# Peterande/SAST

Hardware: AMD Instinct MI355X
Metric: frames/sec (B=4) SAST backbone fwd+bwd, 1Mpx 640x360 (higher is better)
Workload: dtype f32; 1 GPU; 1Mpx 640x360 (padded 384x640) full SAST backbone + PAFPN, fwd+bwd + AdamW, B=4/GPU, binary events (rand>0.5), random-init, AMP=0.0002; global_batch=4, seq_len=1, parallelism=dp1, hipgraph=True, library=sast_amd/libsast_hip.so, product_library=True, segmented_backward_overlap=False, deferred_weight_gradients=False, backward_cuts=3, dw_discard_TIMING_PROBE_gradients_invalid=False, collective_ranks=1, collective_ranks_verified=1, gradient_bytes_per_rank=67663616, sync_batchnorm=False, event_dtype=int32, grads_finite=True

## Files before the change

### sast_amd/csrc/gemm.cuh

```cuda
#pragma once
#include <type_traits>
#include <hip/hip_ext.h>
#include "common.cuh"
#include "../../include/sast_hip.h"

#if defined(SAST_TL_ENABLE) && !defined(SAST_TL)
static __device__ unsigned long long sast_tl_buf[8 * 8192];
#define SAST_TL(k)                                                                                          \
  do {                                                                                                      \
    const unsigned bid_ = blockIdx.x;                                                                       \
    if (threadIdx.x == 0 && bid_ < 8192) sast_tl_buf[bid_ * 8 + (k)] = wall_clock64();                      \
    if (threadIdx.x == 0 && bid_ < 8192 && (k) == 0) sast_tl_buf[bid_ * 8 + 7] = __smid();                 \
  } while (0)
#define SAST_TL_JOB(j) do { if (threadIdx.x == 0 && blockIdx.x < 8192) sast_tl_buf[blockIdx.x * 8 + 6] = (j); } while (0)
#endif
#ifndef SAST_TL
#define SAST_TL(k)
#endif
#ifndef SAST_TL_JOB
#define SAST_TL_JOB(j)
#endif
#ifndef SAST_TLF
#define SAST_TLF_DECL
#define SAST_TLF(k)
// ... 739 lines not shown
  const int remap = xcd_remap_enabled() && nb >= 16;
  const int grid = remap ? (nb + 7) / 8 * 8 : nb;
  if (prof_enabled()) {
    hipEvent_t e0, e1;
    prof_kernel_events(__PRETTY_FUNCTION__, T::G, M, NJ, R, dM, dR, st, &e0, &e1, LoaderSrcBytes<LA>::get(la), LoaderSrcBytes<LB>::get(lb));
    SAST_EXT_LAUNCH((gemm_kernel<T, LA, LB, EP, false>), dim3(grid + ep_side_blocks(ep)), dim3(T::NT), 0, st, e0, e1, 0, la, lb, ep, M, NJ,
                          R, dM, dR, (float*)nullptr, 1, remap);
  } else {
    SAST_LAUNCH((gemm_kernel<T, LA, LB, EP, false>), dim3(grid + ep_side_blocks(ep)), dim3(T::NT), 0, st, la, lb, ep, M, NJ, R, dM, dR,
                       (float*)nullptr, 1, remap);
  }
  SAST_CHECK_LAUNCH();
  return SAST_OK;
}

template <class T, class LA, class LB, class EP>
inline int launch_gemm_split(const LA& la, const LB& lb, const EP& ep, int M, int NJ, int R, const int* dR,
                             int splits, float* colsum, hipStream_t st) {
  if (M <= 0 || NJ <= 0 || R <= 0) return SAST_OK;
  if (colsum != nullptr && LA::RC && GemmSmem<T, LA, LB>::PSA) return SAST_EINVAL;
  if (!gemm_span_ok<T>(la, lb, M, NJ, R)) return SAST_EINVAL;
  const int nb = ((M + T::BM - 1) / T::BM) * ((NJ + T::BJ - 1) / T::BJ);
  if (splits < 1) splits = 1;
  const int remap = xcd_remap_enabled() && nb * splits >= 16;
  const int grid = remap ? (nb * splits + 7) / 8 * 8 : nb * splits;
  if (prof_enabled()) {
    hipEvent_t e0, e1;
    prof_kernel_events(__PRETTY_FUNCTION__, T::G, M, NJ, R, nullptr, dR, st, &e0, &e1, LoaderSrcBytes<LA>::get(la), LoaderSrcBytes<LB>::get(lb));
    SAST_EXT_LAUNCH((gemm_kernel<T, LA, LB, EP, true>), dim3(grid), dim3(T::NT), 0, st, e0, e1, 0, la, lb, ep, M, NJ, R,
                          (const int*)nullptr, dR, colsum, splits, remap);
  } else {
    SAST_LAUNCH((gemm_kernel<T, LA, LB, EP, true>), dim3(grid), dim3(T::NT), 0, st, la, lb, ep, M, NJ, R,
                       (const int*)nullptr, dR, colsum, splits, remap);
  }
  SAST_CHECK_LAUNCH();
  return SAST_OK;
}

inline int gemm_grid(int ntile, int nsplit, int& remap) {
  const int n = ntile * nsplit;
  remap = xcd_remap_enabled() && n >= 16;
  return remap ? (n + 7) / 8 * 8 : n;
}
void prof_kernel_events2(const char* tag, double flops_static, int G1, int M1, int NJ1, int R1, const int* dM1, const int* dR1, int G2,
                         int M2, int NJ2, int R2, const int* dM2, const int* dR2, hipStream_t st, hipEvent_t* e0, hipEvent_t* e1,
                         double a1_cap = -1.0, double b1_cap = -1.0, double a2_cap = -1.0, double b2_cap = -1.0);

template <class TS, class LA1, class LB1, class EP1, class TP, class LA2, class LB2, class EP2>
inline int launch_gemm_dual(const LA1& la1, const LB1& lb1, const EP1& ep1, int M1, int NJ1, int R1, const int* dR1, int splits,
                            float* colsum, const LA2& la2, const LB2& lb2, const EP2& ep2, int M2, int NJ2, int R2, const int* dM2,
                            hipStream_t st) {
  using J1 = GemmJob<TS, LA1, LB1, EP1, true>;
  using J2 = GemmJob<TP, LA2, LB2, EP2, false>;
  if (colsum != nullptr && LA1::RC && GemmSmem<TS, LA1, LB1>::PSA) return SAST_EINVAL;
  if (!gemm_span_ok<TS>(la1, lb1, M1, NJ1, R1) || !gemm_span_ok<TP>(la2, lb2, M2, NJ2, R2)) return SAST_EINVAL;
  if (splits < 1) splits = 1;
  const int nt1 = ((M1 + TS::BM - 1) / TS::BM) * ((NJ1 + TS::BJ - 1) / TS::BJ);
  const int nt2 = ((M2 + TP::BM - 1) / TP::BM) * ((NJ2 + TP::BJ - 1) / TP::BJ);
  int r1, r2;
  int n1 = gemm_grid(nt1, splits, r1);
  const int n2 = gemm_grid(nt2, 1, r2);
  if (r2 && (n1 & 7)) n1 = (n1 + 7) / 8 * 8;
  const J1 a{la1, lb1, ep1, M1, NJ1, R1, nullptr, dR1, colsum, splits, r1};
  const J2 b{la2, lb2, ep2, M2, NJ2, R2, dM2, nullptr, nullptr, 1, r2};
  constexpr int NTHREADS = TS::NT > TP::NT ? TS::NT : TP::NT;
  if (prof_enabled()) {
    hipEvent_t e0, e1;
    prof_kernel_events2(__PRETTY_FUNCTION__, 0.0, TS::G, M1, NJ1, R1, nullptr, dR1, TP::G, M2, NJ2, R2, dM2, nullptr, st, &e0, &e1,
                        LoaderSrcBytes<LA1>::get(la1), LoaderSrcBytes<LB1>::get(lb1), LoaderSrcBytes<LA2>::get(la2), LoaderSrcBytes<LB2>::get(lb2));
    SAST_EXT_LAUNCH((gemm_dual_kernel<J1, J2>), dim3(n1 + n2 + ep_side_blocks(ep2)), dim3(NTHREADS), 0, st, e0, e1, 0, a, b, n1);
  } else {
    SAST_LAUNCH((gemm_dual_kernel<J1, J2>), dim3(n1 + n2 + ep_side_blocks(ep2)), dim3(NTHREADS), 0, st, a, b, n1);
  }
  SAST_CHECK_LAUNCH();
  return SAST_OK;
}

using TileBig   = Tile<128, 128, 2, 2, 1>;
using TileMid   = Tile<64, 128, 2, 2, 1>;
using TileSmall = Tile<64, 64, 2, 2, 1>;
using TileSmallK2 = Tile<64, 64, 2, 2, 1, 16, 2>;
using TileSmallK4 = Tile<64, 64, 2, 2, 1, 16, 4>;
using TileSplitR = Tile<64, 64, 2, 1, 1, 16, 2>;
using TileThinK4  = Tile<32, 64, 1, 2, 1, 16, 4>;
using TileTinyK8 = Tile<32, 32, 1, 1, 1, 16, 8>;
using TileTiny  = Tile<32, 32, 1, 1, 1>;
using TileN64   = Tile<128, 64, 4, 1, 1>;
using TileG2    = Tile<64, 128, 2, 2, 2>;
using TileG2Big = Tile<128, 128, 2, 2, 2>;
using TileG2Tiny = Tile<32, 64, 1, 1, 2>;
using TileG2K2  = Tile<64, 64, 2, 1, 2, 16, 2>;
using TileG2K4  = Tile<32, 64, 1, 1, 2, 16, 4>;
using TileG4K4  = Tile<32, 128, 1, 1, 4, 16, 4>;
using TileG4    = Tile<64, 128, 2, 1, 4, 16, 1, 2, 2>;
using TileG4Big = Tile<128, 128, 4, 1, 4>;
using TileG4Tiny = Tile<32, 128, 1, 1, 4>;
using TileG3    = Tile<64, 96, 2, 1, 3>;
using TileG3K4  = Tile<32, 96, 1, 1, 3, 16, 4>;

__host__ __device__ inline int small_div_mul(int d) { return 65536 / d + 1; }


static __device__ __attribute__((aligned(16))) float sast_zero_page[4];
__device__ __forceinline__ float4 ldz(bool ok, const float* valid) { return ld4(ok ? valid : sast_zero_page); }
__device__ __forceinline__ float ldz1(bool ok, const void* valid) {
  return *reinterpret_cast<const float*>(ok ? valid : (const void*)sast_zero_page);
}
#define SAST_DEFAULT_FINISH \
  __device__ __forceinline__ float4 finish(float4 v, float, bool) const { return v; }

struct LdRows {
  static constexpr bool RC = true, BUFFERED = true;
  const float* p; int ld; const int* idx; int nsrc = 0;
  unsigned long long span_bytes(int I, int, int R) const { return 4ull * ((unsigned long long)((idx ? nsrc : I) - 1) * ld + R); }
  struct Ctx { unsigned row; };
  using Desc = BufDesc;
  __device__ __forceinline__ Desc desc(int) const { return Desc{make_buf(p, BUF_MAX_BYTES)}; }
  __device__ __forceinline__ Ctx prep(int i, int Ieff) const {
    const bool ok = i < Ieff;
    const int ii = ok ? i : 0;
    return Ctx{ok ? 4u * (unsigned)(idx ? idx[ii] : ii) * (unsigned)ld : BUF_INVALID};
  }
  __device__ __forceinline__ void load(const Desc& d, const Ctx& c, int r0, int off, int Rl, int, float4& v, float& aux, bool& ok) const {
    ok = off < Rl - r0;
    v = ldb(d.d, ok ? (c.row + 4u * off) + 4u * r0 : BUF_INVALID);
    aux = 0.f;
  }
  SAST_DEFAULT_FINISH
};
struct LdRows2 {
  static constexpr bool RC = true;
  const float* p1; int ld1; int R1; const float* p2; int ld2;
  struct Ctx { const float* a; const float* b; bool ok; };
  __device__ __forceinline__ Ctx prep(int i, int Ieff) const {
    const bool ok = i < Ieff;
    const int ii = ok ? i : 0;
    return Ctx{p1 + (size_t)ii * ld1, p2 ? p2 + (size_t)ii * ld2 - R1 : p1 + (size_t)ii * ld1, ok};
  }
  __device__ __forceinline__ void load(const Ctx& c, int r, int Reff, float4& v, float& aux, bool& ok) const {
    const bool second = r >= R1;
    ok = c.ok && r < Reff && (!second || p2 != nullptr);
    const float* q = second ? c.b : c.a;
    v = ldz(ok, q + r);
    aux = 0.f;
  }
  SAST_DEFAULT_FINISH
};
struct LdRowsT {
  static constexpr bool RC = false, BUFFERED = true;
  const float* p; int ld;
  unsigned long long span_bytes(int, int, int R) const { return 4ull * (unsigned long long)(R + BUF_SPAN_SLACK_ROWS) * ld; }
  struct Ctx { unsigned col; };
  using Desc = BufDesc;
  __device__ __forceinline__ Desc desc(int Rl) const { return Desc{make_buf(p, 4u * (unsigned)Rl * (unsigned)ld)}; }
  __device__ __forceinline__ Ctx prep(int i, int Ieff) const { return Ctx{i < Ieff ? 4u * i : BUF_INVALID}; }
  __device__ __forceinline__ Ctx prep(int j, int, int NJ) const { return Ctx{j < NJ ? 4u * j : BUF_INVALID}; }
  __device__ __forceinline__ void load(const Desc& d, const Ctx& c, int r0, int off, int, int, float4& v, float& aux, bool& ok) const {
    ok = true;
    v = ldb(d.d, (c.col + 4u * (unsigned)(off * ld)) + 4u * (unsigned)(r0 * ld));
    aux = 0.f;
  }
  SAST_DEFAULT_FINISH
};
struct LdRowsTG {
  static constexpr bool RC = false, BUFFERED = true;
  const float* p; int ld; const int* idx; int nsrc;
// ... 590 lines not shown
```

### sast_amd/csrc/gemm_dispatch.cuh

```cuda
#pragma once
#include <cstdlib>
#include "gemm.cuh"

namespace sast {

using TileAutoThin = TileThinK4;
using TileAutoK2 = TileSmallK2;
using TileAutoK1 = TileSmall;

inline bool gemm_pair_enabled() { return SAST_KNOB("SAST_GEMM_PAIR", 1) != 0; }
inline int pair_tn_blocks() { return SAST_KNOB("SAST_TN_BLOCKS", 768); }
inline int pair_ks_min_r() { return SAST_KNOB("SAST_KS_MINR", 256); }
inline int pair_thin_nb() { return SAST_KNOB("SAST_THIN_NB", 384); }
inline int pair_ks_nb() { return SAST_KNOB("SAST_KS_NB", 1000000); }
inline int tiny_nb() { return SAST_KNOB("SAST_TINY_NB", 128); }
inline bool use_tiny(int M, int NJ, int R) { return (long)((M + 31) / 32) * ((NJ + 63) / 64) <= tiny_nb() && R >= 512; }

template <class LA, class LB, class EP>
int gemm_auto(const LA& la, const LB& lb, const EP& ep, int M, int NJ, int R, const int* dM, hipStream_t st, int R_tile = 0) {
  const long nb = (long)((M + 63) / 64) * ((NJ + 63) / 64);
  const int Rt = R_tile > 0 ? R_tile : R;
  if (!dM && use_tiny(M, NJ, Rt)) return launch_gemm<TileTinyK8>(la, lb, ep, M, NJ, R, dM, nullptr, st);
  if (nb <= pair_thin_nb() && Rt >= pair_ks_min_r()) return launch_gemm<TileAutoThin>(la, lb, ep, M, NJ, R, dM, nullptr, st);
  if (nb <= pair_ks_nb() && Rt >= pair_ks_min_r()) return launch_gemm<TileAutoK2>(la, lb, ep, M, NJ, R, dM, nullptr, st);
  return launch_gemm<TileAutoK1>(la, lb, ep, M, NJ, R, dM, nullptr, st);
}
template <class LA, class LB, class EP>
int gemm_auto(const LA& la, const LB& lb, const EP& ep, int M, int NJ, int R, hipStream_t st) {
  return gemm_auto(la, lb, ep, M, NJ, R, nullptr, st);
}

inline int pair_tn_blocks_conv() { return SAST_KNOB("SAST_TN_BLOCKS_PAIRED_CONV", 192); }
inline int pair_tn_blocks_1x1() { return SAST_KNOB("SAST_TN_BLOCKS_PAIRED_1X1", 192); }
inline int pair_tn_blocks_paired() { return SAST_KNOB("SAST_TN_BLOCKS_PAIRED", 192); }
inline int pair_tn_blocks_small() { return SAST_KNOB("SAST_TN_BLOCKS_PAIRED_SMALL", 0); }
inline int pair_tn_small_tiles() { return SAST_KNOB("SAST_TN_SMALL_TILES", 4); }

inline int tn_splits(int Mo, int NJ, int R, int target = 0) {
  const int nb = ((Mo + 63) / 64) * ((NJ + 63) / 64);
  if (target <= 0) target = pair_tn_blocks();
  int splits = (target + nb - 1) / nb;
  const int max_splits = (R + 127) / 128;
  if (splits > max_splits) splits = max_splits;
  return splits < 1 ? 1 : splits;
}

template <class LA, class LB>
int gemm_tn(const LA& la, const LB& lb, float* out, int ldc, int Mo, int NJ, int R, const int* dR, float* colsum, hipStream_t st) {
  return launch_gemm_split<TileSplitR>(la, lb, EpAtomic{out, ldc}, Mo, NJ, R, dR, tn_splits(Mo, NJ, R), colsum, st);
}
template <class LA, class LB>
int gemm_tn(const LA& la, const LB& lb, float* out, int ldc, int Mo, int NJ, int R, hipStream_t st) {
  return gemm_tn(la, lb, out, ldc, Mo, NJ, R, nullptr, nullptr, st);
}

template <class LA1, class LB1, class EP1, class LA2, class LB2, class EP2>
int gemm_pair_ep(const LA1& la1, const LB1& lb1, const EP1& ep1, int Mo, int NJ1, int R1, const int* dR1, float* colsum,
                 const LA2& la2, const LB2& lb2, const EP2& ep2, int M2, int NJ2, int R2, const int* dM2, hipStream_t st, int tn_target = 0,
                 int R2_tile = 0);
template <class LA1, class LB1, class LA2, class LB2, class EP2>
int gemm_pair(const LA1& la1, const LB1& lb1, float* out, int ldc, int Mo, int NJ1, int R1, const int* dR1, float* colsum,
              const LA2& la2, const LB2& lb2, const EP2& ep2, int M2, int NJ2, int R2, const int* dM2, hipStream_t st, int tn_target = 0,
              int R2_tile = 0) {
  return gemm_pair_ep(la1, lb1, EpAtomic{out, ldc}, Mo, NJ1, R1, dR1, colsum, la2, lb2, ep2, M2, NJ2, R2, dM2, st, tn_target, R2_tile);
}
template <class LA1, class LB1, class EP1, class LA2, class LB2, class EP2>
int gemm_pair_ep(const LA1& la1, const LB1& lb1, const EP1& ep1, int Mo, int NJ1, int R1, const int* dR1, float* colsum,
                 const LA2& la2, const LB2& lb2, const EP2& ep2, int M2, int NJ2, int R2, const int* dM2, hipStream_t st, int tn_target,
                 int R2_tile) {
  const long nb2 = (long)((M2 + 63) / 64) * ((NJ2 + 63) / 64);
  const int R2t = R2_tile > 0 ? R2_tile : R2;
  const bool thin = nb2 <= pair_thin_nb() && R2t >= pair_ks_min_r(), k2 = nb2 <= pair_ks_nb() && R2t >= pair_ks_min_r();
  const int nb1 = ((Mo + 63) / 64) * ((NJ1 + 63) / 64);
  if (gemm_pair_enabled() && pair_tn_blocks_small() > 0 && nb1 <= pair_tn_small_tiles()) tn_target = pair_tn_blocks_small();
  const int splits = tn_splits(Mo, NJ1, R1, gemm_pair_enabled() ? (tn_target > 0 ? tn_target : pair_tn_blocks_paired()) : 0);
  if (!gemm_pair_enabled() || Mo <= 0 || NJ1 <= 0 || R1 <= 0 || M2 <= 0 || NJ2 <= 0 || R2 <= 0) {
    int rc = launch_gemm_split<TileSplitR>(la1, lb1, ep1, Mo, NJ1, R1, dR1, splits, colsum, st);
    if (rc) return rc;
    if (thin) return launch_gemm<TileAutoThin>(la2, lb2, ep2, M2, NJ2, R2, dM2, nullptr, st);
    if (k2) return launch_gemm<TileAutoK2>(la2, lb2, ep2, M2, NJ2, R2, dM2, nullptr, st);
    return launch_gemm<TileAutoK1>(la2, lb2, ep2, M2, NJ2, R2, dM2, nullptr, st);
  }
  if (thin)
    return launch_gemm_dual<TileSplitR, LA1, LB1, EP1, TileAutoThin, LA2, LB2, EP2>(la1, lb1, ep1, Mo, NJ1, R1, dR1, splits, colsum, la2, lb2,
                                                                                      ep2, M2, NJ2, R2, dM2, st);
  if (k2)
    return launch_gemm_dual<TileSplitR, LA1, LB1, EP1, TileAutoK2, LA2, LB2, EP2>(la1, lb1, ep1, Mo, NJ1, R1, dR1, splits, colsum, la2, lb2,
                                                                                       ep2, M2, NJ2, R2, dM2, st);
  return launch_gemm_dual<TileSplitR, LA1, LB1, EP1, TileAutoK1, LA2, LB2, EP2>(la1, lb1, ep1, Mo, NJ1, R1, dR1, splits, colsum, la2, lb2, ep2,
                                                                                   M2, NJ2, R2, dM2, st);
}

}
```

### sast_amd/csrc/k_conv.hip

```cpp
#include <cstdlib>
#include "gemm_dispatch.cuh"
#include "kernels.h"

using namespace sast;

namespace {

inline double bn_unbias(long M) { return M > 1 ? (double)M / (double)(M - 1) : 1.0; }
struct BnFwdJob {
  const float* x; const double* sums; float* run_mean; float* run_var; float* stats; const float* gamma; const float* beta;
  float* y; int ldy; float momentum, eps;
};
__global__ __launch_bounds__(256) void bn_silu_apply_kernel(BnFwdJob j0, BnFwdJob j1, double invM, double unbias, size_t n4, int C, int training, int iters,
                                                            unsigned c4_mul) {
  SAST_KERNARG_WARM_SELF(bn_silu_apply_kernel);
  const BnFwdJob& jb = blockIdx.y == 0 ? j0 : j1;
  const float* __restrict__ x = jb.x; const double* __restrict__ sums = jb.sums;
  float* __restrict__ run_mean = jb.run_mean; float* __restrict__ run_var = jb.run_var; float* __restrict__ stats = jb.stats;
  const float* __restrict__ gamma = jb.gamma; const float* __restrict__ beta = jb.beta; float* __restrict__ y = jb.y;
  const int ldy = jb.ldy; const float momentum = jb.momentum, eps = jb.eps;
  extern __shared__ float bn_sm[];
  const int c4 = C / 4;
  const size_t e0 = (size_t)blockIdx.x * 256 * iters + threadIdx.x;
  for (int c = threadIdx.x; c < C; c += 256) {
// ... 352 lines not shown

template <class LB, class EP>
int conv_gemm(const float* x, const ConvGeom& g, const LB& lb, const EP& ep, int M, int NJ, int K, hipStream_t st) {
  if (!g.cin_mul) return SAST_EINVAL;
  if (g.Cin % 16 == 0) return gemm_auto(LdIm2colU{{x, g}}, lb, ep, M, NJ, K, st);
  return gemm_auto(LdIm2col{x, g}, lb, ep, M, NJ, K, st);
}
template <bool ROWS1, class LB, class EP>
int conv_fwd_gemm(const ConvGeom& g, const LdRows2& src, const LB& lb, const EP& ep, int M, int NJ, int K, hipStream_t st) {
  if (g.KH != 1 || g.stride != 1) return conv_gemm(src.p1, g, lb, ep, M, NJ, K, st);
  if constexpr (ROWS1)
    if (!src.p2) return gemm_auto(LdRows{src.p1, src.ld1, nullptr}, lb, ep, M, NJ, K, st);
  return gemm_auto(src, lb, ep, M, NJ, K, st);
}

int conv_bwd_pair(const float* dconv, const float* x, const ConvGeom& g, int Cout, const float* w, float* dw, float* dx, int lddx,
                  hipStream_t st, const BnProducer* prod = nullptr) {
  const int k = g.KH, K = k * k * g.Cin, M = g.B * g.Ho * g.Wo;
  const unsigned shift = div_mul_of((unsigned)Cout, (unsigned long long)k * k * Cout);
  if (!shift || !g.cin_mul || g.stride_shift < 0) return SAST_EINVAL;
  const LdRowsT ta{dconv, Cout};
  const LdIm2colT tb{x, g};
  if (!dx) return gemm_tn(ta, tb, dw, K, Cout, K, M, st);
  const int parity = SAST_KNOB("SAST_CONVDX_PARITY", 1);
  const int Mc = g.B * (g.H / 2) * (g.W / 2);
  const bool fold = prod && prod->x;
  if (fold && (g.stride != 1 || lddx != g.Cin || prod->C != g.Cin)) return SAST_EINVAL;
  if (fold || !(parity && g.stride == 2 && k == 3 && g.pad == 1 && g.H % 2 == 0 && g.W % 2 == 0 && Mc % 64 == 0))
    return with_dx_epilogue(fold, EpStore{dx, lddx, nullptr}, EpStoreBnRed{dx, lddx, fold ? *prod : BnProducer{}}, [&](const auto& ep) {
      if (Cout % 16 == 0)
        return gemm_pair(ta, tb, dw, K, Cout, K, M, nullptr, nullptr, LdConvDxU{{dconv, g, Cout, Cout, shift}},
                         LdWeightConvDxU{{w, Cout, k * k, g.Cin, shift}}, ep, g.B * g.H * g.W, g.Cin, k * k * Cout, nullptr, st, pair_tn_blocks_conv());
      return gemm_pair(ta, tb, dw, K, Cout, K, M, nullptr, nullptr, LdConvDx{dconv, g, Cout, Cout, shift},
                       LdWeightConvDx{w, Cout, k * k, g.Cin, shift}, ep, g.B * g.H * g.W, g.Cin, k * k * Cout, nullptr, st, pair_tn_blocks_conv());
    });
  ConvDxClasses c;
  c.Hc = g.H / 2; c.Wc = g.W / 2; c.Mc = Mc;
  c.mc_mul = div_mul_of((unsigned)c.Mc, 4ull * Mc); c.wc_mul = div_mul_of((unsigned)c.Wc, 4ull * Mc); c.hc_mul = div_mul_of((unsigned)c.Hc, 4ull * Mc);
  for (int cls = 0; cls < 4; ++cls) {
    const int py = (3 - cls) >> 1, px = (3 - cls) & 1;
    int ty[2] = {15, 15}, tx[2] = {15, 15}, ny = 0, nx = 0;
    for (int kk = 0; kk < k; ++kk) {
      if ((py + g.pad - kk) % 2 == 0 || (g.replicate && py == 0 && kk < g.pad)) ty[ny++] = kk;
      if ((px + g.pad - kk) % 2 == 0 || (g.replicate && px == 0 && kk < g.pad)) tx[nx++] = kk;
    }
    c.kh_pack[cls] = c.kw_pack[cls] = 0;
    int slot = 0;
    for (int pass = 0; pass < 2; ++pass)
      for (int a = 0; a < 2; ++a)
        for (int b = 0; b < 2; ++b) {
          const bool used = ty[a] != 15 && tx[b] != 15;
          if (used != (pass == 0)) continue;
          c.kh_pack[cls] |= (unsigned)(used ? ty[a] : 15) << (4 * slot);
          c.kw_pack[cls] |= (unsigned)(used ? tx[b] : 15) << (4 * slot);
          ++slot;
        }
    c.nslot[cls] = ny * nx;
  }
  return gemm_pair(ta, tb, dw, K, Cout, K, M, nullptr, nullptr, LdConvDxP{dconv, g, Cout, Cout, shift, c},
                   LdWeightConvDxP{w, Cout, k * k, g.Cin, shift, g.KW, c}, EpStoreClass{dx, lddx, g.H, g.W, c}, 4 * Mc, g.Cin, 4 * Cout,
                   nullptr, st, pair_tn_blocks_conv());
}

inline bool stem_exact_bf16() { return SAST_KNOB("SAST_STEM_EXACT_BF16", 1) != 0; }
bool down_size_ok(const SastDownArgs* a) {
  if (a->factor < 1 || a->B < 1 || a->H < a->factor || a->W < a->factor) return false;
  return a->no_overlap || (a->H % a->factor == 0 && a->W % a->factor == 0);
}

}

extern "C" {

int sast_downsample_ln_fwd(const SastDownArgs* a, sast_stream_t stream) { SAST_ENTRY();
  hipStream_t st = (hipStream_t)stream;
  ProfScope ps_("down_fwd", a ? a->Cout : 0, a ? a->B * a->H * a->W : 0, st);
  if (!a || a->Cin % 4 || a->Cout % 4 || !down_size_ok(a)) return SAST_EINVAL;
  const int k = a->no_overlap ? a->factor : 2 * a->factor - 1;
  const ConvGeom g = geom_of(a->B, a->H, a->W, a->Cin, k, a->factor, a->no_overlap ? 0 : a->factor - 1, 1, a->Cin);
  const int M = a->B * g.Ho * g.Wo, K = k * k * a->Cin;
  int rc;
  const bool exact_ok = stem_exact_bf16();
  if (a->x_dtype == SAST_DT_U8 && exact_ok)
    rc = !g.cin_mul ? SAST_EINVAL : gemm_auto(LdIm2colQ8X{{(const unsigned char*)a->x, g}}, LdWeightNT{a->w, K, 0}, EpStore{a->conv_out, a->Cout, nullptr}, M, a->Cout, K, st);
  else if (a->x_dtype == SAST_DT_U8)
    rc = !g.cin_mul ? SAST_EINVAL : gemm_auto(LdIm2colQ8{(const unsigned char*)a->x, g}, LdWeightNT{a->w, K, 0}, EpStore{a->conv_out, a->Cout, nullptr}, M, a->Cout, K, st);
  else if (a->x_dtype != SAST_DT_F32) return SAST_EINVAL;
  else if (a->x_nonexact && exact_ok && g.Cin % 16)
    rc = !g.cin_mul ? SAST_EINVAL : gemm_auto(LdIm2colX{{a->x, g}, a->x_nonexact}, LdWeightNT{a->w, K, 0}, EpStore{a->conv_out, a->Cout, nullptr}, M, a->Cout, K, st);
  else rc = conv_gemm(a->x, g, LdWeightNT{a->w, K, 0}, EpStore{a->conv_out, a->Cout, nullptr}, M, a->Cout, K, st);
  if (rc) return rc;
  return ln_fwd_launch(a->conv_out, a->y, a->ln_w, a->ln_b, a->pe, g.Ho * g.Wo, a->mean, a->rstd, M, a->Cout, 1e-5f, st);
}

int sast_downsample_ln_bwd(const SastDownArgs* a, sast_stream_t stream) { SAST_ENTRY();
  hipStream_t st = (hipStream_t)stream;
  ProfScope ps_("down_bwd", a->Cout, a->B * a->H * a->W, st);
  if (a->Cin % 4 || a->Cout % 4 || !down_size_ok(a) || (a->x_dtype == SAST_DT_U8 && a->dx)) return SAST_EINVAL;
  const int k = a->no_overlap ? a->factor : 2 * a->factor - 1;
  const ConvGeom g = geom_of(a->B, a->H, a->W, a->Cin, k, a->factor, a->no_overlap ? 0 : a->factor - 1, 1, a->Cin);
  const int M = a->B * g.Ho * g.Wo, K = k * k * a->Cin;
  float* dconv = a->ws;
  int rc = ln_bwd_launch(a->conv_out, a->dy, a->ln_w, a->mean, a->rstd, dconv, a->d_ln_w, a->d_ln_b, M, a->Cout, st);
  if (rc) return rc;
  if (a->x_dtype == SAST_DT_U8) {
    if (a->dx || !g.cin_mul) return SAST_EINVAL;
    if (stem_exact_bf16()) return gemm_tn(LdRowsT{dconv, a->Cout}, LdIm2colTQ8X{{(const unsigned char*)a->x, g}}, a->dw, K, a->Cout, K, M, st);
    return gemm_tn(LdRowsT{dconv, a->Cout}, LdIm2colTQ8{(const unsigned char*)a->x, g}, a->dw, K, a->Cout, K, M, st);
  }
  if (a->x_dtype != SAST_DT_F32) return SAST_EINVAL;
  if (a->x_nonexact && !a->dx && stem_exact_bf16() && g.Cin % 16) {
    if (!g.cin_mul) return SAST_EINVAL;
    return gemm_tn(LdRowsT{dconv, a->Cout}, LdIm2colTX{{a->x, g}, a->x_nonexact}, a->dw, K, a->Cout, K, M, st);
  }
  return conv_bwd_pair(dconv, a->x, g, a->Cout, a->w, a->dw, a->dx, a->Cin, st);
}

int sast_conv_bn_ws_floats(int Cout) { SAST_ENTRY(); return SAST_BN_WS_FLOATS(Cout); }

int sast_conv_bn_silu_fwd(const SastConvBnArgs* a, sast_stream_t stream) { SAST_ENTRY();
  hipStream_t st = (hipStream_t)stream;
  ProfScope ps_("convbn_fwd", a ? a->Cout * 10 + a->ksize : 0, a ? a->B * a->H * a->W : 0, st);
  if (!a || a->Cin % 4 || a->Cout % 4 || (a->ksize != 1 && a->ksize != 3)) return SAST_EINVAL;
  const int k = a->ksize, pad = (k - 1) / 2;
  const ConvGeom g = geom_of(a->B, a->H, a->W, a->Cin, k, a->stride, pad, 0, a->ldx);
  const int M = a->B * g.Ho * g.Wo, K = k * k * a->Cin, C = a->Cout;
  if ((unsigned long long)M * (C / 4) >= (1ull << 31)) return SAST_EINVAL;
  const bool dw = a->groups > 1;
  if (dw && (a->groups != a->Cin || a->Cin != a->Cout || a->x2 || a->ldx != a->Cin)) return SAST_EINVAL;
  const DwGeom dg{a->H, a->W, g.Ho, g.Wo, C, k, a->stride};
  double* sums = (double*)a->bn_ws;
  const int phase = a->training ? a->sync_phase : 0;
  if (phase < 0 || phase > 2 || (phase == 2 && a->m_total < M)) return SAST_EINVAL;
  if (a->training && !a->bn_ws_zeroed && phase != 2) zero_fill(a->bn_ws, sizeof(float) * SAST_BN_WS_FLOATS(C), st);
  int rc = SAST_OK;
  const int sep = SAST_KNOB("SAST_BN_STATS_SEPARATE", 0);
  const bool one = k == 1 && a->stride == 1;
  if (a->x2 && (!one || a->Cin1 % 4 || a->Cin1 <= 0 || a->Cin1 >= a->Cin)) return SAST_EINVAL;
  const LdRows2 src{a->x, a->ldx, a->Cin1, a->x2, a->ldx2};
  const LdWeightNT lw{a->w, K, 0};
  if (!a->training && !a->conv_out) {
    if (!a->run_mean || !a->run_var) return SAST_EINVAL;
    if (dw) {
      if (a->ldy != C) return SAST_EINVAL;
      const DwBnSilu bn{a->run_mean, a->run_var, a->bn_w, a->bn_b, a->eps};
      rc = dwconv_fwd_launch(a->x, a->w, nullptr, a->y, a->B, dg, &bn, st);
      if (rc) return rc;
      SAST_CHECK_LAUNCH();
      return SAST_OK;
    }
    return conv_fwd_gemm<true>(g, src, lw, EpBnSilu{a->y, a->ldy, a->run_mean, a->run_var, a->bn_w, a->bn_b, a->eps}, M, C, K, st);
  }
  if (phase == 2) {
  } else if (dw) {
    rc = dwconv_fwd_launch(a->x, a->w, nullptr, a->conv_out, a->B, dg, nullptr, st);
    if (!rc && a->training) bn_stats_launch(a->conv_out, M, C, sums, 128, st);
  } else if (a->training && !sep) {
    rc = conv_fwd_gemm<true>(g, src, lw, EpStoreStats{a->conv_out, C, sums}, M, C, K, st);
  } else {
    rc = conv_fwd_gemm<true>(g, src, lw, EpStore{a->conv_out, C, nullptr}, M, C, K, st);
  }
  if (rc) return rc;
  if (a->training && sep && phase != 2 && !dw) bn_stats_launch(a->conv_out, M, C, sums, sep, st);
  if (phase == 1) { SAST_CHECK_LAUNCH(); return SAST_OK; }
  const BnFwdJob jb{a->conv_out, sums, a->run_mean, a->run_var, a->stats, a->bn_w, a->bn_b, a->y, a->ldy, a->momentum, a->eps};
  bn_fwd_apply_launch(jb, jb, 1, M, phase == 2 ? a->m_total : M, C, a->training, st);
  SAST_CHECK_LAUNCH();
  return SAST_OK;
}

int sast_conv_bn_silu_bwd(const SastConvBnArgs* a, sast_stream_t stream) { SAST_ENTRY();
  hipStream_t st = (hipStream_t)stream;
// ... 201 lines not shown
```

### sast_amd/csrc/k_rows.hip

```cpp
#include <cstdlib>
#include "common.cuh"
#include "kernels.h"

namespace sast {

__global__ __launch_bounds__(256) void zero_fill_kernel(float* __restrict__ p, size_t n) {
  const size_t i = (size_t)blockIdx.x * 256 + threadIdx.x;
  if (i < n) p[i] = 0.f;
}
int zero_fill(void* p, size_t bytes, hipStream_t st) {
  const size_t n = (bytes + 3) / 4;
  if (!n) return SAST_OK;
  SAST_LAUNCH(zero_fill_kernel, dim3((unsigned)((n + 255) / 256)), dim3(256), 0, st, (float*)p, n);
  SAST_CHECK_LAUNCH();
  return SAST_OK;
}

template <typename T>
__global__ __launch_bounds__(256) void nzr_count_kernel(const T* __restrict__ x, int* __restrict__ cnt, int C, int H, int W) {
  __shared__ float cell[8][33];
  const int plane = blockIdx.z;
  const int cy = threadIdx.x >> 5, cx = threadIdx.x & 31;
  const int y0 = blockIdx.y * 32 + cy * 4;
  int n1 = 0, n2 = 0, n3 = 0, n4 = 0;
// ... 13 lines not shown
    }
    __syncthreads();
    cell[cy][cx] = mx;
    n1 += __popcll(__ballot(valid && mx != 0.f));
    __syncthreads();
    bool v2 = false, v3 = false, v4 = false;
    float a = -INFINITY;
    if (threadIdx.x < 64) {
      const int yy = threadIdx.x >> 4, xx = threadIdx.x & 15;
      a = fmaxf(fmaxf(cell[2 * yy][2 * xx], cell[2 * yy][2 * xx + 1]), fmaxf(cell[2 * yy + 1][2 * xx], cell[2 * yy + 1][2 * xx + 1]));
      v2 = (blockIdx.y * 32 + yy * 8 < H) && (xb * 128 + xx * 8 < W);
    }
    __syncthreads();
    if (threadIdx.x < 64) cell[threadIdx.x >> 4][threadIdx.x & 15] = a;
    const unsigned long long m2 = __ballot(v2 && a != 0.f);
    __syncthreads();
    float a3 = -INFINITY;
    if (threadIdx.x < 16) {
      const int yy = threadIdx.x >> 3, xx = threadIdx.x & 7;
      a3 = fmaxf(fmaxf(cell[2 * yy][2 * xx], cell[2 * yy][2 * xx + 1]), fmaxf(cell[2 * yy + 1][2 * xx], cell[2 * yy + 1][2 * xx + 1]));
      v3 = (blockIdx.y * 32 + yy * 16 < H) && (xb * 128 + xx * 16 < W);
    }
    __syncthreads();
    if (threadIdx.x < 16) cell[threadIdx.x >> 3][threadIdx.x & 7] = a3;
    const unsigned long long m3 = __ballot(v3 && a3 != 0.f);
    __syncthreads();
    float a4 = -INFINITY;
    if (threadIdx.x < 4) {
      const int xx = threadIdx.x;
      a4 = fmaxf(fmaxf(cell[0][2 * xx], cell[0][2 * xx + 1]), fmaxf(cell[1][2 * xx], cell[1][2 * xx + 1]));
      v4 = (blockIdx.y * 32 < H) && (xb * 128 + xx * 32 < W);
    }
    const unsigned long long m4 = __ballot(v4 && a4 != 0.f);
    if (threadIdx.x < 64) { n2 += __popcll(m2); n3 += __popcll(m3); n4 += __popcll(m4); }
  }
  const int b = plane / C, c = plane % C;
  int* out = cnt + ((size_t)b * 4) * C + c;
  if ((threadIdx.x & 63) == 0) {
    if (n1) atomicAdd(out + 0 * C, n1);
    if (threadIdx.x == 0) {
      if (n2) atomicAdd(out + 1 * C, n2);
      if (n3) atomicAdd(out + 2 * C, n3);
      if (n4) atomicAdd(out + 3 * C, n4);
    }
  }
}

__global__ void nzr_finish_kernel(const int* __restrict__ cnt, float* __restrict__ r, int n, int C, float s0, float s1, float s2, float s3) {
  const int i = blockIdx.x * blockDim.x + threadIdx.x;
  if (i >= n) return;
  const int lvl = (i / C) & 3;
  const float s = lvl == 0 ? s0 : lvl == 1 ? s1 : lvl == 2 ? s2 : s3;
  r[i] = s * (float)cnt[i];
}

template <typename T>
int nzr_launch(const void* x, int* cnt, float* r, int B, int C, int H, int W, int Hp, int Wp, hipStream_t st) {
  zero_fill(cnt, sizeof(int) * B * 4 * C, st);
  dim3 grid(1, (H + 31) / 32, B * C);
  SAST_LAUNCH((nzr_count_kernel<T>), grid, dim3(256), 0, st, (const T*)x, cnt, C, H, W);
  float s[4];
  int f = 4;
  for (int l = 0; l < 4; ++l) {
    const double numel = (double)B * C * (Hp / f) * (Wp / f);
    s[l] = (float)((double)B / numel);
    f *= 2;
  }
  const int n = B * 4 * C;
  SAST_LAUNCH(nzr_finish_kernel, dim3((n + 255) / 256), dim3(256), 0, st, cnt, r, n, C, s[0], s[1], s[2], s[3]);
  SAST_CHECK_LAUNCH();
  return SAST_OK;
}

int nzr_dispatch(const void* x, int dtype, int* cnt, float* r, int B, int C, int H, int W, int Hp, int Wp, hipStream_t st) {
  switch (dtype) {
    case SAST_DT_F32: return nzr_launch<float>(x, cnt, r, B, C, H, W, Hp, Wp, st);
    case SAST_DT_I32: return nzr_launch<int>(x, cnt, r, B, C, H, W, Hp, Wp, st);
    case SAST_DT_U8:  return nzr_launch<unsigned char>(x, cnt, r, B, C, H, W, Hp, Wp, st);
    case SAST_DT_I8:  return nzr_launch<signed char>(x, cnt, r, B, C, H, W, Hp, Wp, st);
    default: return SAST_EINVAL;
  }
}

constexpr int PREP_WAVES = 2;
template <typename T, int C, typename TY = float>
__global__ __launch_bounds__(64 * PREP_WAVES) void input_prep_kernel(const T* __restrict__ x, TY* __restrict__ y, int* __restrict__ ws,
                                                                     float* __restrict__ r, int B, int H, int W, int Hp, int Wp,
                                                                     float s0, float s1, float s2, float s3,
                                                                     unsigned* __restrict__ nonexact) {
  __shared__ __attribute__((aligned(16))) TY tile_s[PREP_WAVES][8 * 32 * C];
  unsigned low = 0u;
  constexpr bool BYTES = sizeof(TY) == 1;
  __shared__ int cnt_s[4 * C];
  __shared__ int last;
  const int lane = threadIdx.x & 63, wave = threadIdx.x >> 6;
  for (int i = threadIdx.x; i < 4 * C; i += 64 * PREP_WAVES) cnt_s[i] = 0;
  const int tiles_x = Wp / 32, tiles_y = Hp / 32;
  const int tile = blockIdx.x * PREP_WAVES + wave;
  const bool live = tile < B * tiles_y * tiles_x;
  const int tt = live ? tile : 0;
  const int tx = tt % tiles_x, ty = (tt / tiles_x) % tiles_y, b = tt / (tiles_x * tiles_y);
  const int cy = lane >> 3, cx = lane & 7;
  const int y0 = ty * 32 + cy * 4, x0 = tx * 32 + cx * 4;
  const bool inside = live && y0 < H && x0 < W;
  struct alignas(4 * sizeof(T)) Vec4 { T v[4]; };
  TY* tl = tile_s[wave];
  float m[C];
#pragma unroll
  for (int c = 0; c < C; ++c) m[c] = -INFINITY;
  Vec4 q[C];
  auto request = [&](int rr) {
#pragma unroll
    for (int c = 0; c < C; ++c)
      q[c] = *reinterpret_cast<const Vec4*>(x + (((size_t)b * C + c) * H + (inside ? y0 + rr : 0)) * W + (inside ? x0 : 0));
  };
  request(0);
  for (int rr = 0; rr < 4; ++rr) {
    __syncthreads();
#pragma unroll
    for (int c0 = 0; c0 < C; c0 += 4) {
      float v[4][4];
#pragma unroll
      for (int ch = 0; ch < 4; ++ch)
#pragma unroll
        for (int px = 0; px < 4; ++px) {
          v[ch][px] = inside ? (float)q[c0 + ch].v[px] : 0.f;
          if constexpr (!BYTES) low |= __float_as_uint(v[ch][px]);
          m[c0 + ch] = fmaxf(m[c0 + ch], v[ch][px]);
        }
#pragma unroll
      for (int px = 0; px < 4; ++px) {
        if constexpr (BYTES) {
          const unsigned w = inside ? ((unsigned)q[c0].v[px] | ((unsigned)q[c0 + 1].v[px] << 8) | ((unsigned)q[c0 + 2].v[px] << 16) |
                                       ((unsigned)q[c0 + 3].v[px] << 24)) : 0u;
          *reinterpret_cast<unsigned*>(tl + ((cy * 32 + cx * 4 + px) * C + c0)) = w;
        } else {
          st4((float*)tl + ((cy * 32 + cx * 4 + px) * C + c0), make_float4(v[0][px], v[1][px], v[2][px], v[3][px]));
        }
      }
    }
    if (rr < 3) request(rr + 1);
    __syncthreads();
    if (live) {
      constexpr int VE = 16 / sizeof(TY);
      constexpr int ROW4 = 32 * C / VE;
      for (int i = lane; i < 8 * ROW4; i += 64) {
        const int row = i / ROW4, off = i - row * ROW4;
        *reinterpret_cast<float4*>(y + (((size_t)b * Hp + ty * 32 + row * 4 + rr) * Wp + tx * 32) * C + VE * off) =
            *reinterpret_cast<const float4*>(tl + row * 32 * C + VE * off);
      }
    }
  }
#pragma unroll
  for (int c = 0; c < C; ++c) {
    const float mc = m[c];
    const unsigned long long b1 = __ballot(inside && mc != 0.f);
    float m2 = fmaxf(mc, __shfl_xor(mc, 1, 64));  m2 = fmaxf(m2, __shfl_xor(m2, 8, 64));
    float m3 = fmaxf(m2, __shfl_xor(m2, 2, 64)); m3 = fmaxf(m3, __shfl_xor(m3, 16, 64));
    float m4 = fmaxf(m3, __shfl_xor(m3, 4, 64)); m4 = fmaxf(m4, __shfl_xor(m4, 32, 64));
    const unsigned long long b2 = __ballot(!(lane & 9) && inside && m2 != 0.f);
    const unsigned long long b3 = __ballot(!(lane & 27) && inside && m3 != 0.f);
    const unsigned long long b4 = __ballot(lane == 0 && inside && m4 != 0.f);
    if (lane == 0) {
      if (b1) atomicAdd(&cnt_s[0 * C + c], __popcll(b1));
      if (b2) atomicAdd(&cnt_s[1 * C + c], __popcll(b2));
      if (b3) atomicAdd(&cnt_s[2 * C + c], __popcll(b3));
      if (b4) atomicAdd(&cnt_s[3 * C + c], __popcll(b4));
    }
  }
  __syncthreads();
  const int b_blk = (blockIdx.x * PREP_WAVES) / (tiles_x * tiles_y);
  int* cnt = ws;
  if (b_blk < B)
    for (int i = threadIdx.x; i < 4 * C; i += 64 * PREP_WAVES) if (cnt_s[i]) atomicAdd(cnt + (size_t)b_blk * 4 * C + i, cnt_s[i]);
  if constexpr (!BYTES) {
    if (nonexact) {
      const unsigned long long any = __ballot((low & 0xffffu) != 0u);
      if (lane == 0 && any) atomicOr(reinterpret_cast<unsigned*>(ws) + B * 4 * C + 1, 1u);
    }
  }
  __threadfence();
  __syncthreads();
  if (threadIdx.x == 0) last = atomicAdd(ws + B * 4 * C, 1) == (int)gridDim.x - 1;
  __syncthreads();
  if (last) {
    __threadfence();
    for (int i = threadIdx.x; i < B * 4 * C; i += 64 * PREP_WAVES) {
      const int lvl = (i / C) & 3;
      const int n = __hip_atomic_load(cnt + i, __ATOMIC_RELAXED, __HIP_MEMORY_SCOPE_AGENT);
      r[i] = (lvl == 0 ? s0 : lvl == 1 ? s1 : lvl == 2 ? s2 : s3) * (float)n;
      cnt[i] = 0;
    }
    if (threadIdx.x == 0) ws[B * 4 * C] = 0;
    if constexpr (!BYTES) {
      if (nonexact && threadIdx.x == 0) {
        unsigned* word = reinterpret_cast<unsigned*>(ws) + B * 4 * C + 1;
        *nonexact = __hip_atomic_load(word, __ATOMIC_RELAXED, __HIP_MEMORY_SCOPE_AGENT);
        *word = 0u;
      }
    }
  }
}

template <typename T, typename TY = float>
int input_prep_launch(const void* x, TY* y, int* ws, float* r, int B, int C, int H, int W, int Hp, int Wp, hipStream_t st, unsigned* nonexact = nullptr) {
  if (C != 20) return SAST_EINVAL;
  const int tiles = B * (Hp / 32) * (Wp / 32);
  float s[4];
  int f = 4;
  for (int l = 0; l < 4; ++l) {
    const double numel = (double)B * C * (Hp / f) * (Wp / f);
    s[l] = (float)((double)B / numel);
    f *= 2;
  }
  SAST_LAUNCH((input_prep_kernel<T, 20, TY>), dim3((tiles + PREP_WAVES - 1) / PREP_WAVES), dim3(64 * PREP_WAVES), 0, st, (const T*)x, y, ws, r,
                     B, H, W, Hp, Wp, s[0], s[1], s[2], s[3], nonexact);
  SAST_CHECK_LAUNCH();
  return SAST_OK;
}
int input_prep_u8(const unsigned char* x, unsigned char* y, int* ws, float* r, int B, int C, int H, int W, int Hp, int Wp, hipStream_t st) {
  return input_prep_launch<unsigned char, unsigned char>(x, y, ws, r, B, C, H, W, Hp, Wp, st);
}
int input_prep_dispatch(const void* x, int dtype, float* y, int* ws, float* r, int B, int C, int H, int W, int Hp, int Wp, hipStream_t st,
                        unsigned* nonexact) {
  switch (dtype) {
    case SAST_DT_F32: return input_prep_launch<float>(x, y, ws, r, B, C, H, W, Hp, Wp, st, nonexact);
    case SAST_DT_I32: return input_prep_launch<int>(x, y, ws, r, B, C, H, W, Hp, Wp, st, nonexact);
    case SAST_DT_U8:  return input_prep_launch<unsigned char>(x, y, ws, r, B, C, H, W, Hp, Wp, st, nonexact);
    case SAST_DT_I8:  return input_prep_launch<signed char>(x, y, ws, r, B, C, H, W, Hp, Wp, st, nonexact);
    default: return SAST_EINVAL;
  }
}

template <typename T>
__global__ __launch_bounds__(256) void nchw_to_nhwc_kernel(const T* __restrict__ x, float* __restrict__ y, int C, int H, int W, int Hp,
                                                           int Wp, unsigned c_mul) {
  extern __shared__ float tile[];
  const int b = blockIdx.y, p0 = blockIdx.x * 64, HWp = Hp * Wp;
  const int ldt = C + 1;
  const int py0 = p0 / Wp, px0 = p0 - py0 * Wp;
  for (int e = threadIdx.x; e < 64 * C; e += 256) {
    const int c = e >> 6, i = e & 63, p = p0 + i;
    if (p < HWp) {
      int py = py0, px = px0 + i;
      while (px >= Wp) { px -= Wp; ++py; }
      tile[i * ldt + c] = (py < H && px < W) ? (float)x[(((size_t)b * C + c) * H + py) * W + px] : 0.f;
    }
  }
  __syncthreads();
  const int np = min(64, HWp - p0);
  float* o = y + ((size_t)b * HWp + p0) * C;
  for (int e = threadIdx.x; e < np * C; e += 256) {
    const int q = fast_div(e, C, c_mul);
    o[e] = tile[q * ldt + (e - q * C)];
  }
}

int nchw_to_nhwc_dispatch(const void* x, int dtype, float* y, int B, int C, int H, int W, int Hp, int Wp, hipStream_t st) {
  dim3 grid((Hp * Wp + 63) / 64, B);
  const size_t sh = sizeof(float) * 64 * (C + 1);
  switch (dtype) {
    case SAST_DT_F32: SAST_LAUNCH((nchw_to_nhwc_kernel<float>), grid, dim3(256), sh, st, (const float*)x, y, C, H, W, Hp, Wp, div_mul_of((unsigned)C, 64ull * C)); break;
    case SAST_DT_I32: SAST_LAUNCH((nchw_to_nhwc_kernel<int>), grid, dim3(256), sh, st, (const int*)x, y, C, H, W, Hp, Wp, div_mul_of((unsigned)C, 64ull * C)); break;
    case SAST_DT_U8:  SAST_LAUNCH((nchw_to_nhwc_kernel<unsigned char>), grid, dim3(256), sh, st, (const unsigned char*)x, y, C, H, W, Hp, Wp, div_mul_of((unsigned)C, 64ull * C)); break;
    case SAST_DT_I8:  SAST_LAUNCH((nchw_to_nhwc_kernel<signed char>), grid, dim3(256), sh, st, (const signed char*)x, y, C, H, W, Hp, Wp, div_mul_of((unsigned)C, 64ull * C)); break;
    default: return SAST_EINVAL;
  }
  SAST_CHECK_LAUNCH();
  return SAST_OK;
}

__global__ __launch_bounds__(256) void nhwc_to_nchw_kernel(const float* __restrict__ x, float* __restrict__ y, int C, int HW) {
  __shared__ float tile[64][65];
  const int b = blockIdx.z, p0 = blockIdx.x * 64, c0 = blockIdx.y * 64;
  for (int e = threadIdx.x; e < 64 * 64; e += 256) {
    const int p = e >> 6, c = e & 63;
    if (p0 + p < HW && c0 + c < C) tile[p][c] = x[((size_t)b * HW + p0 + p) * C + c0 + c];
  }
  __syncthreads();
  for (int e = threadIdx.x; e < 64 * 64; e += 256) {
    const int c = e >> 6, p = e & 63;
    if (p0 + p < HW && c0 + c < C) y[((size_t)b * C + c0 + c) * HW + p0 + p] = tile[p][c];
  }
}
int nhwc_to_nchw_launch(const float* x, float* y, int B, int C, int HW, hipStream_t st) {
  dim3 grid((HW + 63) / 64, (C + 63) / 64, B);
  SAST_LAUNCH(nhwc_to_nchw_kernel, grid, dim3(256), 0, st, x, y, C, HW);
  SAST_CHECK_LAUNCH();
  return SAST_OK;
}

template <int GL, int VPL>
struct RowIO {
  static constexpr int C = GL * VPL * 4;
  static constexpr int ROWS_PER_WAVE = 64 / GL;
  __device__ static void load(const float* p, float4 (&v)[VPL], int gl) {
#pragma unroll
    for (int i = 0; i < VPL; ++i) v[i] = ld4(p + (i * GL + gl) * 4);
  }
// ... 794 lines not shown
```

Before: 932.6 frames/s.

## Split input-prep tiles across four waves and add tall K2 tile for exact-bf16 stem

The input prep kernel now assigns each 32x32 tile to four waves, one per row phase, instead of one wave looping over four rows. Each wave syncs only within itself, and per-channel maxima are combined through LDS before the ballot counting. The per-block global threadfence is replaced by consuming the atomic return values, which removes a full fence. Separately, the exact-bf16 stem conv GEMM gets a 128x64 split-K2 tile path, meant to raise per-block work. These add LDS reuse tricks and memory-ordering assumptions around the last-block reduction.

After: 937.3 frames/s (median of 6 runs). About the same (+0.5%).

```diff
diff --git a/sast_amd/csrc/gemm.cuh b/sast_amd/csrc/gemm.cuh
--- a/sast_amd/csrc/gemm.cuh
+++ b/sast_amd/csrc/gemm.cuh
@@ -845,6 +845,7 @@
 using TileSmallK2 = Tile<64, 64, 2, 2, 1, 16, 2>;
 using TileSmallK4 = Tile<64, 64, 2, 2, 1, 16, 4>;
 using TileSplitR = Tile<64, 64, 2, 1, 1, 16, 2>;
+using TileTallK2 = Tile<128, 64, 2, 2, 1, 16, 2>;
 using TileThinK4  = Tile<32, 64, 1, 2, 1, 16, 4>;
 using TileTinyK8 = Tile<32, 32, 1, 1, 1, 16, 8>;
 using TileTiny  = Tile<32, 32, 1, 1, 1>;
diff --git a/sast_amd/csrc/gemm_dispatch.cuh b/sast_amd/csrc/gemm_dispatch.cuh
--- a/sast_amd/csrc/gemm_dispatch.cuh
+++ b/sast_amd/csrc/gemm_dispatch.cuh
@@ -28,6 +28,16 @@
 template <class LA, class LB, class EP>
 int gemm_auto(const LA& la, const LB& lb, const EP& ep, int M, int NJ, int R, hipStream_t st) {
   return gemm_auto(la, lb, ep, M, NJ, R, nullptr, st);
+}
+
+inline bool stem_tall_tile() { return SAST_KNOB("SAST_STEM_TALL_TILE", 1) != 0; }
+template <class LA, class LB, class EP>
+int gemm_auto_exact_a(const LA& la, const LB& lb, const EP& ep, int M, int NJ, int R, hipStream_t st) {
+  static_assert(LoaderExactBf16<LA>::value, "A must carry the EXACT_BF16 trait");
+  const long nb = (long)((M + 63) / 64) * ((NJ + 63) / 64);
+  const bool k2 = !use_tiny(M, NJ, R) && nb > pair_thin_nb() && nb <= pair_ks_nb() && R >= pair_ks_min_r();
+  if (k2 && stem_tall_tile()) return launch_gemm<TileTallK2>(la, lb, ep, M, NJ, R, nullptr, nullptr, st);
+  return gemm_auto(la, lb, ep, M, NJ, R, st);
 }
 
 inline int pair_tn_blocks_conv() { return SAST_KNOB("SAST_TN_BLOCKS_PAIRED_CONV", 192); }
diff --git a/sast_amd/csrc/k_conv.hip b/sast_amd/csrc/k_conv.hip
--- a/sast_amd/csrc/k_conv.hip
+++ b/sast_amd/csrc/k_conv.hip
@@ -458,12 +458,12 @@
   int rc;
   const bool exact_ok = stem_exact_bf16();
   if (a->x_dtype == SAST_DT_U8 && exact_ok)
-    rc = !g.cin_mul ? SAST_EINVAL : gemm_auto(LdIm2colQ8X{{(const unsigned char*)a->x, g}}, LdWeightNT{a->w, K, 0}, EpStore{a->conv_out, a->Cout, nullptr}, M, a->Cout, K, st);
+    rc = !g.cin_mul ? SAST_EINVAL : gemm_auto_exact_a(LdIm2colQ8X{{(const unsigned char*)a->x, g}}, LdWeightNT{a->w, K, 0}, EpStore{a->conv_out, a->Cout, nullptr}, M, a->Cout, K, st);
   else if (a->x_dtype == SAST_DT_U8)
     rc = !g.cin_mul ? SAST_EINVAL : gemm_auto(LdIm2colQ8{(const unsigned char*)a->x, g}, LdWeightNT{a->w, K, 0}, EpStore{a->conv_out, a->Cout, nullptr}, M, a->Cout, K, st);
   else if (a->x_dtype != SAST_DT_F32) return SAST_EINVAL;
   else if (a->x_nonexact && exact_ok && g.Cin % 16)
-    rc = !g.cin_mul ? SAST_EINVAL : gemm_auto(LdIm2colX{{a->x, g}, a->x_nonexact}, LdWeightNT{a->w, K, 0}, EpStore{a->conv_out, a->Cout, nullptr}, M, a->Cout, K, st);
+    rc = !g.cin_mul ? SAST_EINVAL : gemm_auto_exact_a(LdIm2colX{{a->x, g}, a->x_nonexact}, LdWeightNT{a->w, K, 0}, EpStore{a->conv_out, a->Cout, nullptr}, M, a->Cout, K, st);
   else rc = conv_gemm(a->x, g, LdWeightNT{a->w, K, 0}, EpStore{a->conv_out, a->Cout, nullptr}, M, a->Cout, K, st);
   if (rc) return rc;
   return ln_fwd_launch(a->conv_out, a->y, a->ln_w, a->ln_b, a->pe, g.Ho * g.Wo, a->mean, a->rstd, M, a->Cout, 1e-5f, st);
diff --git a/sast_amd/csrc/k_rows.hip b/sast_amd/csrc/k_rows.hip
--- a/sast_amd/csrc/k_rows.hip
+++ b/sast_amd/csrc/k_rows.hip
@@ -119,21 +119,29 @@
   }
 }
 
-constexpr int PREP_WAVES = 2;
+constexpr int PREP_WAVES = 4;
+constexpr int PREP_TILES = 2;
 template <typename T, int C, typename TY = float>
-__global__ __launch_bounds__(64 * PREP_WAVES) void input_prep_kernel(const T* __restrict__ x, TY* __restrict__ y, int* __restrict__ ws,
+__global__ __launch_bounds__(64 * PREP_WAVES * PREP_TILES, 4) void input_prep_kernel(const T* __restrict__ x, TY* __restrict__ y, int* __restrict__ ws,
                                                                      float* __restrict__ r, int B, int H, int W, int Hp, int Wp,
                                                                      float s0, float s1, float s2, float s3,
                                                                      unsigned* __restrict__ nonexact) {
-  __shared__ __attribute__((aligned(16))) TY tile_s[PREP_WAVES][8 * 32 * C];
+  constexpr bool BYTES = sizeof(TY) == 1;
+  constexpr int TPW = PREP_TILES;
+  constexpr int PH_ROWS = BYTES ? 8 : 4;
+  constexpr int WAVE_LDS = PH_ROWS * 32 * C * (int)sizeof(TY);
+  static_assert(WAVE_LDS >= 64 * C * (int)sizeof(float), "the staging tile also carries the wave's row maxima");
+  __shared__ __attribute__((aligned(16))) unsigned char tile_s[TPW * PREP_WAVES][WAVE_LDS];
+  constexpr int NT = 64 * PREP_WAVES * TPW;
   unsigned low = 0u;
-  constexpr bool BYTES = sizeof(TY) == 1;
-  __shared__ int cnt_s[4 * C];
-  __shared__ int last;
+  constexpr bool CNT_IN_TILE = WAVE_LDS >= (64 * C + 4 * C + 1) * (int)sizeof(int);
+  __shared__ int cnt_own[CNT_IN_TILE ? 1 : 4 * C + 1];
+  int* cnt_s = CNT_IN_TILE ? reinterpret_cast<int*>(tile_s[0]) + 64 * C : cnt_own;
+  int& last = cnt_s[4 * C];
   const int lane = threadIdx.x & 63, wave = threadIdx.x >> 6;
-  for (int i = threadIdx.x; i < 4 * C; i += 64 * PREP_WAVES) cnt_s[i] = 0;
   const int tiles_x = Wp / 32, tiles_y = Hp / 32;
-  const int tile = blockIdx.x * PREP_WAVES + wave;
+  const int tw = wave / PREP_WAVES, rr = wave % PREP_WAVES;
+  const int tile = blockIdx.x * TPW + tw;
   const bool live = tile < B * tiles_y * tiles_x;
   const int tt = live ? tile : 0;
   const int tx = tt % tiles_x, ty = (tt / tiles_x) % tiles_y, b = tt / (tiles_x * tiles_y);
@@ -141,56 +149,64 @@
   const int y0 = ty * 32 + cy * 4, x0 = tx * 32 + cx * 4;
   const bool inside = live && y0 < H && x0 < W;
   struct alignas(4 * sizeof(T)) Vec4 { T v[4]; };
-  TY* tl = tile_s[wave];
+  TY* tl = reinterpret_cast<TY*>(tile_s[wave]);
   float m[C];
 #pragma unroll
   for (int c = 0; c < C; ++c) m[c] = -INFINITY;
   Vec4 q[C];
-  auto request = [&](int rr) {
-#pragma unroll
-    for (int c = 0; c < C; ++c)
-      q[c] = *reinterpret_cast<const Vec4*>(x + (((size_t)b * C + c) * H + (inside ? y0 + rr : 0)) * W + (inside ? x0 : 0));
-  };
-  request(0);
-  for (int rr = 0; rr < 4; ++rr) {
-    __syncthreads();
-#pragma unroll
-    for (int c0 = 0; c0 < C; c0 += 4) {
-      float v[4][4];
-#pragma unroll
-      for (int ch = 0; ch < 4; ++ch)
+#pragma unroll
+  for (int c = 0; c < C; ++c)
+    q[c] = *reinterpret_cast<const Vec4*>(x + (((size_t)b * C + c) * H + (inside ? y0 + rr : 0)) * W + (inside ? x0 : 0));
+  auto wave_sync = [] { __builtin_amdgcn_fence(__ATOMIC_ACQ_REL, "wavefront"); __builtin_amdgcn_wave_barrier(); };
+#pragma unroll
+  for (int ph = 0; ph < 8 / PH_ROWS; ++ph) {
+    if (ph) wave_sync();
+    if (cy / PH_ROWS == ph) {
+      const int ry = cy % PH_ROWS;
+#pragma unroll
+      for (int c0 = 0; c0 < C; c0 += 4) {
+        float v[4][4];
+#pragma unroll
+        for (int ch = 0; ch < 4; ++ch)
+#pragma unroll
+          for (int px = 0; px < 4; ++px) {
+            v[ch][px] = inside ? (float)q[c0 + ch].v[px] : 0.f;
+            if constexpr (!BYTES) low |= __float_as_uint(v[ch][px]);
+            m[c0 + ch] = fmaxf(m[c0 + ch], v[ch][px]);
+          }
 #pragma unroll
         for (int px = 0; px < 4; ++px) {
-          v[ch][px] = inside ? (float)q[c0 + ch].v[px] : 0.f;
-          if constexpr (!BYTES) low |= __float_as_uint(v[ch][px]);
-          m[c0 + ch] = fmaxf(m[c0 + ch], v[ch][px]);
-        }
-#pragma unroll
-      for (int px = 0; px < 4; ++px) {
-        if constexpr (BYTES) {
-          const unsigned w = inside ? ((unsigned)q[c0].v[px] | ((unsigned)q[c0 + 1].v[px] << 8) | ((unsigned)q[c0 + 2].v[px] << 16) |
-                                       ((unsigned)q[c0 + 3].v[px] << 24)) : 0u;
-          *reinterpret_cast<unsigned*>(tl + ((cy * 32 + cx * 4 + px) * C + c0)) = w;
-        } else {
-          st4((float*)tl + ((cy * 32 + cx * 4 + px) * C + c0), make_float4(v[0][px], v[1][px], v[2][px], v[3][px]));
+          if constexpr (BYTES) {
+            const unsigned w = inside ? ((unsigned)q[c0].v[px] | ((unsigned)q[c0 + 1].v[px] << 8) | ((unsigned)q[c0 + 2].v[px] << 16) |
+                                         ((unsigned)q[c0 + 3].v[px] << 24)) : 0u;
+            *reinterpret_cast<unsigned*>(tl + ((ry * 32 + cx * 4 + px) * C + c0)) = w;
+          } else {
+            st4((float*)tl + ((ry * 32 + cx * 4 + px) * C + c0), make_float4(v[0][px], v[1][px], v[2][px], v[3][px]));
+          }
         }
       }
     }
-    if (rr < 3) request(rr + 1);
-    __syncthreads();
-    if (live) {
-      constexpr int VE = 16 / sizeof(TY);
-      constexpr int ROW4 = 32 * C / VE;
-      for (int i = lane; i < 8 * ROW4; i += 64) {
-        const int row = i / ROW4, off = i - row * ROW4;
-        *reinterpret_cast<float4*>(y + (((size_t)b * Hp + ty * 32 + row * 4 + rr) * Wp + tx * 32) * C + VE * off) =
-            *reinterpret_cast<const float4*>(tl + row * 32 * C + VE * off);
-      }
-    }
-  }
-#pragma unroll
-  for (int c = 0; c < C; ++c) {
-    const float mc = m[c];
+    wave_sync();
+    constexpr int VE = 16 / sizeof(TY);
+    constexpr int ROW4 = 32 * C / VE;
+    if (live)
+    for (int i = lane; i < PH_ROWS * ROW4; i += 64) {
+      const int row = i / ROW4, off = i - row * ROW4;
+      *reinterpret_cast<float4*>(y + (((size_t)b * Hp + ty * 32 + (ph * PH_ROWS + row) * 4 + rr) * Wp + tx * 32) * C + VE * off) =
+          *reinterpret_cast<const float4*>(tl + row * 32 * C + VE * off);
+    }
+  }
+  wave_sync();
+  float* ms = reinterpret_cast<float*>(tile_s[wave]);
+#pragma unroll
+  for (int c = 0; c < C; ++c) ms[c * 64 + lane] = m[c];
+  if (wave == 0)
+    for (int i = lane; i < 4 * C; i += 64) cnt_s[i] = 0;
+  __syncthreads();
+  for (int c = rr; c < C; c += PREP_WAVES) {
+    const float* m0 = reinterpret_cast<const float*>(tile_s[tw * PREP_WAVES]) + c * 64 + lane;
+    constexpr int WS = WAVE_LDS / (int)sizeof(float);
+    const float mc = fmaxf(fmaxf(m0[0], m0[WS]), fmaxf(m0[2 * WS], m0[3 * WS]));
     const unsigned long long b1 = __ballot(inside && mc != 0.f);
     float m2 = fmaxf(mc, __shfl_xor(mc, 1, 64));  m2 = fmaxf(m2, __shfl_xor(m2, 8, 64));
     float m3 = fmaxf(m2, __shfl_xor(m2, 2, 64)); m3 = fmaxf(m3, __shfl_xor(m3, 16, 64));
@@ -206,23 +222,24 @@
     }
   }
   __syncthreads();
-  const int b_blk = (blockIdx.x * PREP_WAVES) / (tiles_x * tiles_y);
+  const int b_blk = (blockIdx.x * TPW) / (tiles_x * tiles_y);
   int* cnt = ws;
+  int seen = 0;
   if (b_blk < B)
-    for (int i = threadIdx.x; i < 4 * C; i += 64 * PREP_WAVES) if (cnt_s[i]) atomicAdd(cnt + (size_t)b_blk * 4 * C + i, cnt_s[i]);
+    for (int i = threadIdx.x; i < 4 * C; i += NT) if (cnt_s[i]) seen |= atomicAdd(cnt + (size_t)b_blk * 4 * C + i, cnt_s[i]);
   if constexpr (!BYTES) {
     if (nonexact) {
       const unsigned long long any = __ballot((low & 0xffffu) != 0u);
-      if (lane == 0 && any) atomicOr(reinterpret_cast<unsigned*>(ws) + B * 4 * C + 1, 1u);
-    }
-  }
-  __threadfence();
+      if (lane == 0 && any) seen |= (int)atomicOr(reinterpret_cast<unsigned*>(ws) + B * 4 * C + 1, 1u);
+    }
+  }
+  asm volatile("" ::"v"(seen) : "memory");
   __syncthreads();
   if (threadIdx.x == 0) last = atomicAdd(ws + B * 4 * C, 1) == (int)gridDim.x - 1;
   __syncthreads();
   if (last) {
     __threadfence();
-    for (int i = threadIdx.x; i < B * 4 * C; i += 64 * PREP_WAVES) {
+    for (int i = threadIdx.x; i < B * 4 * C; i += NT) {
       const int lvl = (i / C) & 3;
       const int n = __hip_atomic_load(cnt + i, __ATOMIC_RELAXED, __HIP_MEMORY_SCOPE_AGENT);
       r[i] = (lvl == 0 ? s0 : lvl == 1 ? s1 : lvl == 2 ? s2 : s3) * (float)n;
@@ -250,8 +267,8 @@
     s[l] = (float)((double)B / numel);
     f *= 2;
   }
-  SAST_LAUNCH((input_prep_kernel<T, 20, TY>), dim3((tiles + PREP_WAVES - 1) / PREP_WAVES), dim3(64 * PREP_WAVES), 0, st, (const T*)x, y, ws, r,
-                     B, H, W, Hp, Wp, s[0], s[1], s[2], s[3], nonexact);
+  SAST_LAUNCH((input_prep_kernel<T, 20, TY>), dim3((tiles + PREP_TILES - 1) / PREP_TILES), dim3(64 * PREP_WAVES * PREP_TILES), 0, st, (const T*)x, y,
+                     ws, r, B, H, W, Hp, Wp, s[0], s[1], s[2], s[3], nonexact);
   SAST_CHECK_LAUNCH();
   return SAST_OK;
 }
```
